# VKoskiv/c-ray

Hardware: AMD Instinct MI355X
Metric: Mray/s (primary+secondary) (higher is better)
Workload: dtype f32; 1 GPU; input/hdr.json 1280x720, 256 spp, 8 bounces (BASELINE.json configs[1]); venusscaled.obj = generated 524288-triangle stand-in (tools/gen_assets.py), HDR env map + 2048^2 grid texture from the reference tree; environment map: a generated stand-in of the HDR's size (tools/cfg2_blob.py — no reference tree to flatten hdr.json from): the same paths and rays, other radiance; parallelism=1 rank: the whole frame in one dispatch

## Files before the change

### c-ray_amd/csrc/cray_hip.hip

```cpp
#include <hip/hip_runtime.h>
#include <dlfcn.h>

#include <algorithm>
#include <chrono>
#include <cmath>
#include <cstdio>
#include <cstring>
#include <condition_variable>
#include <atomic>
#include <cassert>
#include <memory>
#include <mutex>
#include <thread>
#include <string>
#include <vector>

#include "cray_hip.h"
#define CRH_EM_POW_TABLES_IN_LDS
#include "pt_device.h"
#include "scene_compile.h"
#include "ctx_access.h"

using namespace crh;

// ... 6 lines not shown
#endif
#define CRH_INST_LDS_BYTES ((CRH_INST_LDS0_MAX + CRH_INST_LDS1_MAX) * 64u)
#ifndef CRH_SHADE_LDS
#define CRH_SHADE_LDS 1
#endif
#define CRH_SHADE_LDS_MATERIALS 24u
#define CRH_SHADE_LDS_BSDFS 64u
#define CRH_SHADE_LDS_CONSTS 48u
#define CRH_SHADE_LDS_IMAGES 8u
#define CRH_SHADE_LDS_BYTES (CRH_SHADE_LDS * (CRH_SHADE_LDS_MATERIALS * 32u + CRH_SHADE_LDS_BSDFS * 16u + CRH_SHADE_LDS_CONSTS * 16u + CRH_SHADE_LDS_IMAGES * 40u))
#ifndef CRH_STACK_LDS
#define CRH_STACK_LDS ((40960 - 3968 - (int)CRH_INST_LDS_BYTES - (int)CRH_SHADE_LDS_BYTES) / 1024 - 15)
#endif
#ifndef CRH_LOCKSTEP
#define CRH_LOCKSTEP() do { } while (0)
#endif

static thread_local std::string t_err;
static int fail(int code, const std::string &msg) { t_err = msg; return code; }
#define HIP_TRY(expr)                                                                               \
	do {                                                                                            \
		hipError_t e_ = (expr);                                                                     \
		if (e_ != hipSuccess) return fail(CRH_ERR_HIP, std::string(#expr) + ": " + hipGetErrorString(e_)); \
	} while (0)
#include "ctx_buffers.h"

#define CRH_STACK_OVF (134 - CRH_STACK_LDS)
#define CRH_OVF_WORDS_PER_WAVE (128u * 64u)
typedef __attribute__((address_space(3))) uint32_t lds_u32;
typedef __attribute__((address_space(1))) uint32_t glb_u32;
// ... 104 lines not shown
};

template <class T>
__device__ __forceinline__ const T *asGlobal(const T *p) {
	return (const T *)(const __attribute__((address_space(1))) T *)p;
}
__device__ __forceinline__ DScene globalize(const DScene &S) {
	DScene G = S;
	G.nodes = asGlobal(S.nodes); G.tris = asGlobal(S.tris); G.prims = asGlobal(S.prims); G.shade = asGlobal(S.shade);
	G.instances = asGlobal(S.instances); G.materials = asGlobal(S.materials);
	G.bsdfs = asGlobal(S.bsdfs); G.consts = asGlobal(S.consts); G.images = asGlobal(S.images); G.prog = asGlobal(S.prog);
	G.textures = asGlobal(S.textures); G.texels = asGlobal(S.texels);
	G.camera = (const crh_camera *)(const __attribute__((address_space(4))) crh_camera *)S.camera;
	return G;
}

__device__ __forceinline__ uint32_t waveSum(uint32_t v) {
	for (int off = 32; off > 0; off >>= 1) v += __shfl_xor(v, off);
	return v;
}
__device__ __forceinline__ void flushCounter(bool lead, uint32_t laneCount, unsigned long long *counter) {
	const uint32_t v = waveSum(laneCount);
	if (lead && v) atomicAdd(counter, (unsigned long long)v);
}
template <class Cnt>
__device__ __forceinline__ void flushWalkCounters(bool lead, const Cnt &cnt, unsigned long long *counters) {
	flushCounter(lead, cnt.rays, &counters[1]);
	if constexpr (Cnt::level >= 2) {
		flushCounter(lead, cnt.node_tests, &counters[2]);
		flushCounter(lead, cnt.tri_tests, &counters[3]);
// ... 105 lines not shown
		return v;
	}
	__device__ __forceinline__ f4 *at(uint32_t bytes) const { return (f4 *)((char *)base + bytes); }
	__device__ __forceinline__ f4 *rec(uint32_t id) const { return base + id * (LEAN ? 4u : CRH_PATH_F4); }
	__device__ __forceinline__ f4 *hit(uint32_t id) const { return LEAN ? at(vgprConst(CRH_PATHS * 64u) + id * 16u) : base + id * CRH_PATH_F4 + 4u; }
	__device__ __forceinline__ float *inst(uint32_t id) const { return LEAN ? (float *)at(vgprConst(CRH_PATHS * 80u) + id * 4u) : (float *)(base + id * CRH_PATH_F4 + 5u); }
};
static_assert(CRH_PATHS * (4u + 1u) * 4u + CRH_PATHS <= CRH_WAVE_QUEUE_FLOATS, "the lean arrays fit in the wave's table");
static_assert((CRH_WAVE_QUEUE_FLOATS * sizeof(float)) % 64u == 0, "a wave's table starts on a 64-B line when the allocation does, and a lean rec(id) (64 B) is one aligned line: loadRec4 / storeRec4");

__device__ __forceinline__ uint32_t laneRank(unsigned long long m) {
	return __builtin_amdgcn_mbcnt_hi((uint32_t)(m >> 32), __builtin_amdgcn_mbcnt_lo((uint32_t)m, 0u));
}

#if CRH_SHADE_LDS
#define CRH_STAGE_SHADE_TABLES() \
	__shared__ __attribute__((aligned(16))) uint32_t s_shade[CRH_SHADE_LDS_BYTES / 4u]; \
	stk.shadeTab = nullptr; \
	if (S.material_count <= CRH_SHADE_LDS_MATERIALS && S.bsdf_count <= CRH_SHADE_LDS_BSDFS && S.const_count <= CRH_SHADE_LDS_CONSTS && \
		S.image_count <= CRH_SHADE_LDS_IMAGES && S.texture_count <= CRH_SHADE_LDS_IMAGES) { \
		const uint32_t texBase = CRH_SHADE_LDS_MATERIALS * 8u + CRH_SHADE_LDS_BSDFS * 4u + CRH_SHADE_LDS_CONSTS * 4u; \
		for (uint32_t i = threadIdx.x; i < S.texture_count * 8u; i += CRH_BLOCK) s_shade[texBase + i] = ((const uint32_t *)S.textures)[i]; \
		for (uint32_t i = threadIdx.x; i < S.image_count * 2u; i += CRH_BLOCK) s_shade[texBase + CRH_SHADE_LDS_IMAGES * 8u + i] = ((const uint32_t *)S.images)[i]; \
		for (uint32_t i = threadIdx.x; i < S.material_count * 8u; i += CRH_BLOCK) s_shade[i] = ((const uint32_t *)S.materials)[i]; \
		for (uint32_t i = threadIdx.x; i < S.bsdf_count * 4u; i += CRH_BLOCK) s_shade[CRH_SHADE_LDS_MATERIALS * 8u + i] = ((const uint32_t *)S.bsdfs)[i]; \
		for (uint32_t i = threadIdx.x; i < S.const_count * 4u; i += CRH_BLOCK) s_shade[CRH_SHADE_LDS_MATERIALS * 8u + CRH_SHADE_LDS_BSDFS * 4u + i] = ((const uint32_t *)S.consts)[i]; \
		__syncthreads(); \
		stk.shadeTab = (const lds_u32 *)s_shade; \
	}
#else
#define CRH_STAGE_SHADE_TABLES() do { } while (0)
#endif
#if CRH_INST_LDS_BYTES > 0
#define CRH_STAGE_INSTANCE_TABLES() \
	__shared__ __attribute__((aligned(16))) uint32_t s_inst[CRH_INST_LDS_BYTES / 4u]; \
	stk.inst0 = stk.inst1 = nullptr; \
	{ \
		const bool st0 = S.instance_count <= CRH_INST_LDS0_MAX, st1 = S.instance_count <= CRH_INST_LDS1_MAX; \
		if (st0) for (uint32_t i = threadIdx.x; i < S.instance_count * 16u; i += CRH_BLOCK) s_inst[i] = ((const uint32_t *)(S.instances + (i >> 4)))[i & 15u]; \
		if (st1) for (uint32_t i = threadIdx.x; i < S.instance_count * 16u; i += CRH_BLOCK) s_inst[CRH_INST_LDS0_MAX * 16u + i] = ((const uint32_t *)(S.instances + (i >> 4)))[16u + (i & 15u)]; \
		if (st0 || st1) __syncthreads(); \
		if (st0) stk.inst0 = (const lds_u32 *)s_inst; \
		if (st1) stk.inst1 = (const lds_u32 *)s_inst + CRH_INST_LDS0_MAX * 16u; \
	}
#else
#define CRH_STAGE_INSTANCE_TABLES() do { } while (0)
// ... 170 lines not shown
	size_t streamSlots = 0;
	DevBuf<float> dStreamSlab;
	StreamCtl *dStreamCtl = nullptr;
	DevBuf<uint32_t> dStreamOvf;
	unsigned int *hStreamDone = nullptr, *dStreamDone = nullptr;
	unsigned int streamSeq = 0;
	uint64_t streamIterations = 0;
	hipEvent_t streamEv[2] = {nullptr, nullptr};
	uint32_t lastGrid = 0;
	char lastKernel[64] = "";
	DevBuf<float> dStage;
	bool haveScene = false;
	bool hasPrograms = true;
	bool hasVolumes = false;
	DScene d;
	int walk = CRH_WALK_BINARY;
	bool haveWide = false;
	uint32_t wideTlasRoot = 0;
	std::vector<void *> sceneAllocs;
	unsigned long long *dCounters = nullptr;
	uint32_t *dWork = nullptr;
	uint32_t workSlot = 0;
	StagedBuf tileSlots[64];
	std::vector<TimedPair> pendingTimes;
	TimedPool eventPool;
	float lastMs = 0.0f;
	double totalMs = 0.0;
	uint64_t launches = 0;
	uint32_t aovDepth = 0;
	SideDispatch aov;
// ... 14 lines not shown
}

static int watchTimeMs(const char *who, crh_ctx *c, Stopwatch<1> *watch, float *last_ms) {
	if (!c || !last_ms) return fail(CRH_ERR_INVALID, std::string(who) + ": NULL argument");
	int rc = setDevice(c);
	if (rc) return rc;
	if ((rc = watch->read())) return rc;
	*last_ms = watch->sum;
	return CRH_OK;
}

static void freeScene(crh_ctx *c) {
	for (void *p : c->sceneAllocs) (void)hipFree(p);
	c->sceneAllocs.clear();
	c->haveScene = false;
}

static int resolveTimes(crh_ctx *c, bool wait) {
	size_t done = 0;
	for (auto &t : c->pendingTimes) {
		if (wait) HIP_TRY(hipEventSynchronize(t.b));
		else if (hipEventQuery(t.b) != hipSuccess) break;
		float ms = 0.0f;
		HIP_TRY(hipEventElapsedTime(&ms, t.a, t.b));
		c->lastMs = ms;
		c->totalMs += ms;
		c->eventPool.give(t);
		++done;
	}
	c->pendingTimes.erase(c->pendingTimes.begin(), c->pendingTimes.begin() + done);
// ... 81 lines not shown
	CRH_WAVE_ROW(1, 4, true, 0),
#else
	CRH_WAVE_ROW(1, 4, false, 0),
#endif
};
#undef CRH_WAVE_ROW
#endif

static hipError_t launchPathtrace(crh_ctx *c, uint32_t grid, const crh_render_params *P, const BlockQueue &Q, float *dev_fb, int chunk) {
	const int level = c->counterLevel >= 2 ? 2 : 1, samp = c->sampler == CRH_SAMPLER_HALTON ? 1 : 0;
	const char *name = nullptr;
	if (rollForm(c)) {
		const bool wide = wideWalk(c);
		DScene d = c->d;
		if (wide && d.tlas_node_count > 1u) d.tlas_root = c->wideTlasRoot;
		if (const auto *r = pickRow(kRollRows, level, c->hasPrograms, samp, wide ? 1 : 0)) {
			name = r->name;
			hipLaunchKernelGGL((r->fn), dim3(grid), dim3(CRH_BLOCK), 0, c->stream, d, *P, Q, dev_fb, c->dCounters, c->dStage.p, chunk, c->dWaveStats, c->sched, c->dQueues.p, c->dOvf.p, c->dErr);
		}
	}
#ifdef CRH_WITH_ALT_KERNELS
	else if (c->kernel == CRH_KERNEL_WG) {
		if (const auto *r = pickRow(kWgRows, level, c->hasPrograms, samp, 0)) {
			name = r->name;
			hipLaunchKernelGGL((r->fn), dim3(grid), dim3(CRH_BLOCK), 0, c->stream, c->d, *P, Q, dev_fb, c->dCounters, c->dStage.p, chunk, c->schedWg, c->dQueues.p, c->dOvf.p, c->dErr);
		}
	} else if (const auto *r = pickRow(kWaveRows, level, c->hasPrograms, samp, samp || c->wavesPerSimd >= 4 ? 4 : 1)) {
		name = r->name;
		hipLaunchKernelGGL((r->fn), dim3(grid), dim3(CRH_BLOCK), 0, c->stream, c->d, *P, Q, dev_fb, c->dCounters, c->dStage.p, chunk, c->dWaveStats, c->sched, c->dQueues.p, c->dOvf.p);
	}
// ... 71 lines not shown
	crh_ctx *c = new (std::nothrow) crh_ctx();
	if (!c) return fail(CRH_ERR_NOMEM, "out of host memory");
	c->device = device;
	hipError_t e = hipSetDevice(device);
	hipDeviceProp_t prop;
	if (e == hipSuccess) e = hipGetDeviceProperties(&prop, device);
	if (e == hipSuccess) {
		c->cuCount = prop.multiProcessorCount;
		if (stream) c->stream = (hipStream_t)stream;
		else { e = hipStreamCreateWithFlags(&c->stream, hipStreamNonBlocking); c->ownStream = (e == hipSuccess); }
	}
	if (e == hipSuccess) e = hipMalloc((void **)&c->dCounters, CRH_COUNTER_BYTES(c->cuCount));
	if (e == hipSuccess) e = hipMemset(c->dCounters, 0, CRH_COUNTER_BYTES(c->cuCount));
	if (e == hipSuccess) e = hipMalloc((void **)&c->dWork, CRH_WORK_SLOTS * sizeof(uint32_t));
	if (e == hipSuccess) e = hipMemset(c->dWork, 0, CRH_WORK_SLOTS * sizeof(uint32_t));
	if (e == hipSuccess) e = hipHostMalloc((void **)&c->hErr, sizeof(unsigned int), hipHostMallocDefault);
	if (e == hipSuccess) { *c->hErr = 0u; e = hipHostGetDevicePointer((void **)&c->dErr, c->hErr, 0); }
	if (e != hipSuccess) {
		const std::string msg = std::string("crh_context_create: ") + hipGetErrorString(e);
		crh_context_destroy(c);
		return fail(CRH_ERR_HIP, msg);
	}
	const char *env = getenv("CRH_BLOCKS_PER_CU");
	if (env && atoi(env) > 0) c->blocksPerCU = atoi(env) > 8 ? 8 : atoi(env);
	env = getenv("CRH_SWAP_IN_RUN");
	if (env && atoi(env) >= 1 && atoi(env) <= 65) c->sched.swapInRun = atoi(env);
	env = getenv("CRH_KERNEL");
	if (env && !strcmp(env, "stream")) c->kernel = CRH_KERNEL_STREAM;
	if (env && !strcmp(env, "roll")) c->kernel = CRH_KERNEL_ROLL;
	env = getenv("CRH_STREAM_COHORTS");
// ... 13 lines not shown
	}
	if (join && c->janitor.joinable()) c->janitor.join();
}

int crh_context_destroy(crh_ctx *c) {
	if (!c) return CRH_OK;
	(void)hipSetDevice(c->device);
	if (c->stream) (void)hipStreamSynchronize(c->stream);
	freeScene(c);
	auto drop = [](void *p) { if (p) (void)hipFree(p); };
	auto dropEvent = [](hipEvent_t e) { if (e) (void)hipEventDestroy(e); };
	for (StagedBuf &ts : c->tileSlots) ts.release();
	for (const TimedPair &t : c->pendingTimes) c->eventPool.give(t);
	c->pendingTimes.clear();
	c->eventPool.release();
	drop(c->dCounters); drop(c->dWork);
	c->dStage.release(); c->dDefer.release(); c->dQueues.release(); c->dOvf.release();
	for (SideDispatch *s : {&c->aov, &c->ids}) { drop(s->counter); s->tiles.release(); s->watch.release(); }
	c->dPack.release(); c->packWatch.release();
	c->dDenoise.release(); c->denoiseWatch.release();
	c->adaptive.release(); c->adaptiveWatch.release();
	if (c->hErr) (void)hipHostFree(c->hErr);
	if (c->pinned) (void)hipHostFree(c->pinned);
	releaseJanitor(c, true);
	c->dSrgb.release(); c->dGather.release();
	drop(c->dWaveStats); drop(c->dDump);
	for (int i = 0; i < 2; ++i) { drop(c->dProbeHits[i]); drop(c->dProbeInst[i]); }
	drop(c->dProbeOvf); c->dProbeUnits.release();
	c->dStreamPlanes.release(); c->dStreamHit.release(); c->dStreamHitInst.release(); c->dStreamCount.release(); c->dStreamSlab.release();
	drop(c->dStreamCtl); c->dStreamOvf.release();
	if (c->hStreamDone) (void)hipHostFree(c->hStreamDone);
// ... 143 lines not shown
	UP(textures, cs.textures.data(), cs.textures.size());
	{
		void *texDev = nullptr;
		rc = takeTexels ? takeTexels(&texDev) : CRH_OK;
		if (rc) { freeScene(c); return rc; }
		if (texDev) { c->sceneAllocs.push_back(texDev); d.texels = (const f4 *)texDev; }
		else UP(texels, cs.texels.data(), cs.texels.size());
	}
#undef UP
	d.tlas_first = cs.tlas_first;
	d.material_count = (uint32_t)cs.materials.size(); d.bsdf_count = (uint32_t)cs.bsdfs.size(); d.const_count = (uint32_t)cs.consts.size();
	d.image_count = (uint32_t)cs.images.size(); d.texture_count = (uint32_t)cs.textures.size();
	d.tlas_root = cs.tlas_root; d.tlas_node_count = cs.tlas_node_count; d.tlas_prim_base = cs.tlas_prim_base; d.shade_classes = cs.shade_classes; d.instance_count = (uint32_t)cs.instances.size();
	d.background = cs.background;
	{ const crh_camera *cam = nullptr; rc = upload(c, &cs.camera, 1, &cam); if (rc) { freeScene(c); return rc; } d.camera = cam; }
	c->d = d;
	c->haveWide = !cs.wide.empty(); c->wideTlasRoot = cs.wide_tlas_root;
	if (cs.want_wide && !c->haveWide && !cs.wide_refused.empty())
		fprintf(stderr, "libcray_hip: CRH_WALK_WIDE4 was asked for, but this scene has no 4-ary copy (%s): the binary walk renders it\n", cs.wide_refused.c_str());
	c->hasPrograms = cs.prog.size() > 1 || cs.has_volumes || getenv("CRH_FORCE_PROGRAMS") != nullptr;
	c->hasVolumes = cs.has_volumes;
	c->aovDepth = cs.max_albedo_depth;
	c->haveScene = true;
	*tCopiesMs = upMs();
	rc = preloadKernel(c, true);
	if (rc != CRH_OK) return rc;
	unsigned int flag = 0;
	HIP_TRY(hipMemcpy(&flag, c->dWork + (CRH_WORK_SLOTS - 1), sizeof(flag), hipMemcpyDeviceToHost));
	return CRH_OK;
}
// ... 1714 lines not shown
```

### c-ray_amd/csrc/pathtrace_roll.h

```cpp
#pragma once

#define CRH_ROLL_HITS_MAX 136u
#define CRH_ROLL_IDS_MISSES (CRH_IDS_HITS + 2u * CRH_ROLL_HITS_MAX)
#define CRH_ROLL_IDS_BYTES (CRH_ROLL_IDS_MISSES + 128u)
#ifndef CRH_ROLL_SLOTS
#define CRH_ROLL_SLOTS 4u
#endif
#ifndef CRH_ROLL_FIFO
#define CRH_ROLL_FIFO 0
#endif
#define CRH_ROLL_SLOT_SHIFT 30u
#define CRH_ROLL_ITEM_MASK 0x3FFFFFFFu


template <int LEVEL, int WPS, bool PROG, int SAMP, bool WIDE = false>
__global__ __launch_bounds__(CRH_BLOCK, CRH_WPS_OVERRIDE) void k_pathtrace_roll(const DScene Sarg, const crh_render_params P, const BlockQueue Q, float *fb,
																 unsigned long long *counters,
																 float *stage, int chunk, unsigned long long *waveStats, const Sched K, float *queues, uint32_t *ovfAll, unsigned int *errFlag) {
	__shared__ uint32_t s_stack[CRH_STACK_LDS * CRH_BLOCK];
	__shared__ uint32_t s_park[CRH_PARK_SLOTS * CRH_BLOCK];
	enum { RQ_RAYS, RQ_HITS, RQ_MISSES, RQ_FREE, RQ_CLS_LO, RQ_CLS_HI,
	       RQ_GENLEFT,
	       RQ_FLAGS,
	       RQ_HEAD,
// ... 9 lines not shown
#define CRH_RQ_IS_DRY(v) ((v) != 0)
	enum { NS = (int)CRH_ROLL_SLOTS, RQ_WORDS = RQ_SLOT0 + NS * SJ_WORDS };
	static_assert(NS >= 2 && NS <= 4, "2..4 job slots (two bits of the item word)");
	static_assert((CRH_STACK_LDS + CRH_PARK_SLOTS) * CRH_BLOCK * 4 + (CRH_BLOCK / 64) * (CRH_ROLL_IDS_BYTES + RQ_WORDS * 4) + 512 + 256 + CRH_INST_LDS_BYTES + CRH_SHADE_LDS_BYTES <= 40960, "4 blocks per CU share 160 KB of LDS (incl. powf's tables)");
	const DScene S = globalize(Sarg);
	CRH_EM_POW_TABLES_INIT();
	const unsigned long long tStart = wall_clock64();
	uint32_t unitsDone = 0;
#ifdef CRH_EXP_ABS_TIMES
	unsigned long long tDry = 0;
	bool snapDone = false;
#endif
	LdsStack stk;
	stk.lds = (lds_u32 *)&s_stack[threadIdx.x];
	stk.parkp = (lds_u32 *)&s_park[threadIdx.x];
	CRH_STAGE_SHADE_TABLES();
	CRH_STAGE_INSTANCE_TABLES();
	CountersT<LEVEL, PROG, WIDE> cnt;
	memset(&cnt, 0, sizeof(cnt));
	const uint32_t lane = threadIdx.x & 63u;
	const uint32_t wave = (blockIdx.x * CRH_BLOCK + threadIdx.x) >> 6;
	__shared__ uint8_t s_cls[256];
	const bool sorted = K.sortFrom > 0 && S.shade_classes >= (uint32_t)K.sortFrom && S.instance_count <= 256u;
	if (sorted) {
		for (uint32_t i = threadIdx.x; i < S.instance_count; i += CRH_BLOCK) s_cls[i] = (uint8_t)CRH_DINST_CLASS(S.instances[i].kind);
		__syncthreads();
	}
	stk.ovf = (glb_u32 *)ovfAll + (size_t)__builtin_amdgcn_readfirstlane(wave) * CRH_OVF_WORDS_PER_WAVE;
	const size_t slabFloats = (size_t)Q.bw * Q.bh * chunk * 3;
	float *const myStage = stage + (size_t)__builtin_amdgcn_readfirstlane(wave) * (size_t)NS * slabFloats;
	const int passEnd = P.first_pass + P.pass_count;
	const uint32_t trisOff = (uint32_t)((const char *)S.tris - (const char *)S.nodes);
	constexpr bool LEANTAB = CRH_PATH_LEAN && !PROG;
	constexpr bool COOP_LOAD = LEANTAB && CRH_REC_COOP_LOAD == 1, COOP_LOAD_MISS = LEANTAB && CRH_REC_COOP_LOAD >= 1 , COOP_STORE = LEANTAB && CRH_REC_COOP_STORE, MISS_SKIP_HIT = LEANTAB && CRH_MISS_SKIP_HIT;
	const PathTab<LEANTAB> tab{(f4 *)(queues + (size_t)__builtin_amdgcn_readfirstlane(wave) * CRH_WAVE_QUEUE_FLOATS)};
	unsigned long long *const waveCtr = counters + CRH_NCOUNTERS + (size_t)__builtin_amdgcn_readfirstlane(wave) * CRH_NCOUNTERS;
	float *dumpRays = nullptr;
	uint32_t dumpCap = 0, dumpCount = 0;
	if constexpr (LEVEL >= 2) {
		if (waveStats) {
			const unsigned long long base = waveStats[CRH_DUMP_HDR];
			if (base) { dumpCap = (uint32_t)waveStats[CRH_DUMP_HDR + 1]; dumpRays = (float *)(__attribute__((address_space(1))) float *)(uintptr_t)base + (size_t)__builtin_amdgcn_readfirstlane(wave) * dumpCap * 6u; }
		}
	}
#define CRH_WCTR(k, v) atomicAdd(&waveCtr[k], (unsigned long long)(uint32_t)(v))
	__shared__ int s_rq[(CRH_BLOCK / 64) * RQ_WORDS];
	__shared__ __attribute__((aligned(2))) uint8_t s_ids[(CRH_BLOCK / 64) * CRH_ROLL_IDS_BYTES];
	typedef volatile __attribute__((address_space(3))) int lds_int;
// ... 25 lines not shown
			if (left < 0) left = 0;
			moreChunks = !(gj[SJ_WH] & SJ_WH_DEFER) && gj[SJ_PASS0] + gj[SJ_PASSN] < passEnd;
			if (oj[SJ_NEXT] >= (ob & 0xFFFF) * (ob >> 16) * oj[SJ_PASSN] && oj[SJ_OUT] == 0 && (open > 1 || !moreChunks)) flags |= 1;
		}
		if (open < NS && (!CRH_RQ_IS_DRY(wq[RQ_DRY]) || moreChunks)) flags |= 2;
		wq[RQ_GENLEFT] = left; wq[RQ_FLAGS] = flags;
	};

	if (lane == 0) {
		wq[RQ_RAYS] = 0; wq[RQ_HITS] = 0; wq[RQ_MISSES] = 0; wq[RQ_FREE] = (int)CRH_PATHS; wq[RQ_CLS_LO] = 0; wq[RQ_CLS_HI] = 0;
		wq[RQ_HEAD] = 0; wq[RQ_OPEN] = 0; wq[RQ_GEN] = 0; wq[RQ_DRY] = 0;
		for (int i = 0; i < NS * SJ_WORDS; ++i) wq[RQ_SLOT0 + i] = 0;
		refreshJobWords();
	}
	for (uint32_t i = lane; i < CRH_PATHS; i += 64u) ids[i] = (uint8_t)i;
	__threadfence_block();
	Walk w;
	memset(&w, 0, sizeof(w));
	w.phase = PH_IDLE;
	uint32_t myPath = 0;
	auto retireRefill = [&](int &rq, int &hq, int &mq) __attribute__((always_inline)) {
		const bool fin = (w.phase == PH_SHADE);
		const bool finHit = fin && w.hit.inst >= 0, finMiss = fin && w.hit.inst < 0;
		const unsigned long long hm = __ballot(finHit), mm = __ballot(finMiss);
		uint32_t cls = 0;
		if (fin) {
			if (!MISS_SKIP_HIT || finHit) *tab.hit(myPath) = f4{w.hit.t, w.hit.u, w.hit.v, asF32((uint32_t)w.hit.slot)};
			if (finHit) {
				*tab.inst(myPath) = asF32((uint32_t)w.hit.inst);
				if (sorted) cls = (uint32_t)((volatile __attribute__((address_space(3))) uint8_t *)s_cls)[w.hit.inst];
				hits[(uint32_t)hq + laneRank(hm)] = (uint16_t)(myPath | (cls << 8));
// ... 30 lines not shown
			myPath = myRay;
#else
		if (idle && (int)er < take) {
			myPath = ids[CRH_IDS_RAYS + (uint32_t)(rq - take) + er];
#endif
			const f4 *q = tab.rec(myPath);
			const f4 q0 = q[0], q1 = q[1];
			{ TablePort<SAMP> port2{tab.rec(myPath)}; walkBegin(S, w, stk, v3{q0.x, q0.y, q0.z}, v3{q1.x, q1.y, q1.z}, cnt, port2, (uint32_t)K.rayFlags); }
			if constexpr (LEVEL >= 2) {
				if (dumpRays && dumpCount + er < dumpCap) { float *o = dumpRays + (size_t)(dumpCount + er) * 6u; o[0] = q0.x; o[1] = q0.y; o[2] = q0.z; o[3] = q1.x; o[4] = q1.y; o[5] = q1.z; }
			}
		}
		if constexpr (LEVEL >= 2) dumpCount += (uint32_t)take;
		hq += (int)__popcll(hm); mq += (int)__popcll(mm); rq -= take;
		if (lane == 0) { wq[RQ_HITS] = hq; wq[RQ_MISSES] = mq; wq[RQ_RAYS] = rq; }
		__threadfence_block();
	};
	uint32_t guard = (uint32_t)K.roundLimit;
	for (;;) {
		if (--guard == 0u) { if (lane == 0) atomicOr(errFlag, CRH_ERRFLAG_ROUND_LIMIT); break; }
#ifdef CRH_EXP_ABS_TIMES
		if (waveStats && !snapDone && (guard & 15u) == 0u) {
			uint32_t handedOut = 0;
			if (lane == 0) handedOut = __hip_atomic_load((uint32_t *)Q.counter, __ATOMIC_RELAXED, __HIP_MEMORY_SCOPE_AGENT);
			handedOut = __builtin_amdgcn_readfirstlane(handedOut);
			if (handedOut >= Q.total) {
				snapDone = true;
				if (lane == 0) {
					const int head = wq[RQ_HEAD], open = wq[RQ_OPEN];
					unsigned long long notGenerated = 0, notStaged = 0;
					for (int k = 0; k < open; ++k) {
// ... 59 lines not shown
					if constexpr (LEVEL >= 2) {
						if (lane == 0) { CRH_WCTR(11, 1); CRH_WCTR(17, now); }
#ifdef CRH_CENSUS
						const uint32_t wf = (uint32_t)__popcll(__ballot(w.phase == PH_SHADE || w.phase == PH_IDLE));
						if (lane == 0) { CRH_WCTR(30, nTw >= K.triInRun ? 0u : (uint32_t)nTw); CRH_WCTR(31, wf); if (nTw >= K.triInRun) { CRH_WCTR(26, 1); CRH_WCTR(27, nTw); } }
#endif
					}
					if (isN || isT) {
						const uint32_t off = isN ? (uint32_t)(w.node << (WIDE ? 4 : 5)) : trisOff + w.pA * 48u;
						const char *rec = (const char *)S.nodes + off;
						q0 = *(const f4 *)rec; q1 = *(const f4 *)(rec + 16); q2 = *(const f4 *)(rec + 32); q3 = *(const f4 *)(rec + 48);
						if (WIDE || isT) { q4 = *(const f4 *)(rec + 64); q5 = *(const f4 *)(rec + 80); }
						if (WIDE && isN) { q6 = *(const f4 *)(rec + 96); q7 = *(const f4 *)(rec + 112); }
					}
					if constexpr (WIDE) { if (isN) stepWideLoaded<true>(S, w, stk, cnt, port, q0, q1, q2, q3, q4, q5, q6, q7); }
					else
					if (isN) stepNodeLoaded<true>(S, w, stk, cnt, port, q0, q1, q2, q3);
					if (isT) stepTriLoaded(S, w, stk, cnt, port, q0, q1, q2, q3, q4, q5);
					if ((int)__popcll(__ballot(w.phase == PH_CTRL)) >= K.ctrlInRun) {
#ifdef CRH_CENSUS
						if constexpr (LEVEL >= 2) { const uint32_t n2 = (uint32_t)__popcll(__ballot(w.phase == PH_CTRL)); if (lane == 0) { CRH_WCTR(28, 1); CRH_WCTR(29, n2); } }
#endif
						if (w.phase == PH_CTRL) stepCtrl(S, w, stk, cnt, port);
					}
					{
						const int nFi = (int)__popcll(__ballot(w.phase == PH_SHADE)), nEi = (int)__popcll(__ballot(w.phase == PH_IDLE));
						if (nFi + nEi >= K.swapInRun && (nFi > 0 || rqRun > 0) && hqRun < 64 && mqRun < 64) {
							if constexpr (LEVEL >= 2) { if (lane == 0) { CRH_WCTR(21, 1); CRH_WCTR(23, nFi + min(nEi + nFi, rqRun)); } }
							retireRefill(rqRun, hqRun, mqRun);
							port = TablePort<SAMP>{tab.rec(myPath)};
						}
					}
					now = __popcll(__ballot(w.phase == PH_NODE));
// ... 67 lines not shown
					if (have) {
						lds_int *j = wq + RQ_SLOT0 + s * SJ_WORDS;
						j[SJ_X0] = J.x0; j[SJ_Y0] = J.y0; j[SJ_WH] = J.w | (J.h << 16) | defer
						          ; j[SJ_BWBH] = J.bw | (J.bh << 16); j[SJ_PASS0] = J.passBegin; j[SJ_PASSN] = J.passCount;
						j[SJ_NEXT] = 0; j[SJ_OUT] = 0;
						j[SJ_BASE_LO] = (int)(uint32_t)(uintptr_t)base; j[SJ_BASE_HI] = (int)(uint32_t)((uintptr_t)base >> 32);
						wq[RQ_OPEN] = open + 1; wq[RQ_GEN] = s;
					} else {
						wq[RQ_DRY] = 1;
					}
#ifdef CRH_EXP_ABS_TIMES
					if (!have && !tDry) tDry = wall_clock64();
#endif
					refreshJobWords();
				}
				__threadfence_block();
				break;
			}
			case ST_GEN: {
				const int g = wq[RQ_GEN];
				const BlockJob J = loadJob(g);
				const uint32_t genNext = (uint32_t)wq[RQ_SLOT0 + g * SJ_WORDS + SJ_NEXT], genItems = genNext + (uint32_t)itemsLeft;
				const uint32_t item = genNext + lane;
				int x = 0, y = 0, pass = 0;
				const bool valid = item < genItems && decodeItem(J, item, x, y, pass);
				const unsigned long long vm = __ballot(valid);
				const int n = (int)__popcll(vm);
				if constexpr (COOP_STORE) {
					f4 q0 = f4{0.0f, 0.0f, 0.0f, 0.0f}, q1 = q0, q2 = q0, q3 = q0;
					uint32_t id = 0;
					if (valid) {
// ... 10 lines not shown
				if (valid) {
					const uint32_t rk = laneRank(vm);
					const uint32_t id = ids[CRH_IDS_FREE_END - (uint32_t)freeQ + rk];
					v3 ro, rd;
					PathRecT<RngT<SAMP>> r;
					beginPath(S, P, x, y, pass, ro, rd, r, cnt);
					putPathRay(tab.rec(id), ro, rd, r, item | ((uint32_t)g << CRH_ROLL_SLOT_SHIFT));
					ids[CRH_IDS_RAYS + (uint32_t)raysQ + rk] = (uint8_t)id;
				}
				if (lane == 0) {
					wq[RQ_RAYS] = raysQ + n; wq[RQ_FREE] = freeQ - n;
					lds_int *j = wq + RQ_SLOT0 + g * SJ_WORDS;
					j[SJ_NEXT] = (int)(genNext + 64u); j[SJ_OUT] = j[SJ_OUT] + n;
					refreshJobWords();
				}
				__threadfence_block();
				break;
			}
			case ST_MISS: {
				const int n = min(missQn, 64);
				int mySlot = -1;
				const bool have = (int)lane < n;
				uint32_t id = 0;
				f4 q0, q1, q2, q3;
				if constexpr (COOP_LOAD_MISS) {
					if (have) id = ids[CRH_ROLL_IDS_MISSES + (uint32_t)(missQn - n) + lane];
					tab.loadRec4(id, have, q0, q1, q2, q3);
				}
				if (have) {
					if constexpr (!COOP_LOAD_MISS) { id = ids[CRH_ROLL_IDS_MISSES + (uint32_t)(missQn - n) + lane]; const f4 *q = tab.rec(id); q1 = q[1]; q2 = q[2]; q3 = q[3]; }
					v3 ro{0.0f, 0.0f, 0.0f}, rd{q1.x, q1.y, q1.z};
					PathRecT<RngT<SAMP>> r;
					r.wr = q2.x; r.wg = q2.y; r.wb = q2.z;
					r.fr = q3.x; r.fg = q3.y; r.fb = q3.z;
					r.rng.state = 0; r.depth = 0;
					const uint32_t item = asU32(q1.w);
					mySlot = (int)(item >> CRH_ROLL_SLOT_SHIFT);
					TravHit h;
					h.t = MISS_SKIP_HIT ? 0.0f : tab.hit(id)->x; h.u = h.v = 0.0f; h.slot = -1; h.inst = -1;
					(void)shadeCore(S, P, ro, rd, h, r, cnt, stk);
					float *so = sampleSlot(mySlot, item & CRH_ROLL_ITEM_MASK); so[0] = r.fr; so[1] = r.fg; so[2] = r.fb;
					ids[CRH_IDS_FREE_END - 1u - (uint32_t)freeQ - lane] = (uint8_t)id;
				}
				int fin[NS];
#pragma unroll
				for (int s = 0; s < NS; ++s) fin[s] = (int)__popcll(__ballot(mySlot == s));
				if (lane == 0) {
					wq[RQ_MISSES] = missQn - n; wq[RQ_FREE] = freeQ + n;
#pragma unroll
					for (int s = 0; s < NS; ++s) if (fin[s]) wq[RQ_SLOT0 + s * SJ_WORDS + SJ_OUT] = wq[RQ_SLOT0 + s * SJ_WORDS + SJ_OUT] - fin[s];
					refreshJobWords();
				}
				__threadfence_block();
				break;
			}
			case ST_FOLD: {
				const int o = wq[RQ_HEAD], open = wq[RQ_OPEN];
				const BlockJob J = loadJob(o);
				__threadfence_block();
				const float *slab = myStage + (size_t)o * slabFloats;
				if (!jobDeferred(o)) {
					for (uint32_t pix = lane; pix < (uint32_t)(J.bw * J.bh); pix += 64u) foldBlockPixel(P, J, pix, slab, fb);
				}
				__threadfence_block();
				CRH_LOCKSTEP();
				if (lane == 0) { wq[RQ_HEAD] = (o + 1) % NS; wq[RQ_OPEN] = open - 1; refreshJobWords(); }
				__threadfence_block();
				break;
			}
			default: {
				uint32_t clsLo = 0, clsHi = 0;
				int n = min(hitsQ, 64);
				if (sorted) {
				clsLo = (uint32_t)__builtin_amdgcn_readfirstlane(wq[RQ_CLS_LO]); clsHi = (uint32_t)__builtin_amdgcn_readfirstlane(wq[RQ_CLS_HI]);
				int c8[8];
#pragma unroll
				for (int b = 0; b < 8; ++b) c8[b] = (int)(((b < 4 ? clsLo : clsHi) >> (8 * (b & 3))) & 255u);
				uint32_t fullMask = 0;
				int partCls = -1, partN = 0;
				n = 0;
#pragma unroll
				for (int it = 0; it < 8; ++it) {
// ... 54 lines not shown
					if constexpr (!COOP_LOAD) id = (uint32_t)hits[(uint32_t)(hitsQ - n) + lane] & 255u;
					f4 *q = tab.rec(id);
					if constexpr (!COOP_LOAD) { q0 = q[0]; q1 = q[1]; q2 = q[2]; q3 = q[3]; }
					const f4 q4 = *tab.hit(id);
					v3 ro{q0.x, q0.y, q0.z}, rd{q1.x, q1.y, q1.z};
					PathRecT<RngT<SAMP>> r;
					r.wr = q2.x; r.wg = q2.y; r.wb = q2.z;
					r.fr = q3.x; r.fg = q3.y; r.fb = q3.z;
					r.rng.state = (uint64_t)asU32(q2.w) | ((uint64_t)asU32(q3.w) << 32);
					r.depth = (int)asU32(q0.w);
					const uint32_t item = asU32(q1.w);
					TravHit h;
					h.t = q4.x; h.u = q4.y; h.v = q4.z;
					h.slot = (int32_t)asU32(q4.w); h.inst = (int32_t)asU32(*tab.inst(id));
					__builtin_assume(h.inst >= 0);
					cont = shadeCore(S, P, ro, rd, h, r, cnt, stk);
					done = !cont;
					if constexpr (COOP_STORE) packPathRay(q0, q1, q2, q3, ro, rd, r, item);
					else if (cont) putPathRay(q, ro, rd, r, item);
					if (!cont) {
						mySlot = (int)(item >> CRH_ROLL_SLOT_SHIFT);
						float *so = sampleSlot(mySlot, item & CRH_ROLL_ITEM_MASK); so[0] = r.fr; so[1] = r.fg; so[2] = r.fb;
					}
				}
				if constexpr (COOP_STORE) tab.storeRec4(id, cont, q0, q1, q2, q3);
				const unsigned long long cm = __ballot(cont), dm = __ballot(done);
				int fin[NS];
#pragma unroll
				for (int s = 0; s < NS; ++s) fin[s] = (int)__popcll(__ballot(mySlot == s));
				if (cont) ids[CRH_IDS_RAYS + (uint32_t)raysQ + laneRank(cm)] = (uint8_t)id;
				if (done) ids[CRH_IDS_FREE_END - 1u - (uint32_t)freeQ - laneRank(dm)] = (uint8_t)id;
				if (lane == 0) {
					const int nd = (int)__popcll(dm);
					wq[RQ_HITS] = hitsQ - n; wq[RQ_RAYS] = raysQ + (int)__popcll(cm); wq[RQ_FREE] = freeQ + nd;
					wq[RQ_CLS_LO] = (int)clsLo; wq[RQ_CLS_HI] = (int)clsHi;
#pragma unroll
					for (int s = 0; s < NS; ++s) if (fin[s]) wq[RQ_SLOT0 + s * SJ_WORDS + SJ_OUT] = wq[RQ_SLOT0 + s * SJ_WORDS + SJ_OUT] - fin[s];
					if (nd) refreshJobWords();
				}
				__threadfence_block();
				break;
			}
		}
		if constexpr (LEVEL >= 2) {
			if (lane == 0) {
				const uint32_t dt = CRH_TICK() - tk;
				CRH_WCTR(14, 1);
				if (pick == ST_NODE) { CRH_WCTR(9, dt); }
				else if (pick == ST_TRI) { CRH_WCTR(8, dt); }
				else if (pick == ST_CTRL) { CRH_WCTR(13, 1); CRH_WCTR(16, dt); CRH_WCTR(25, nC); }
				else if (pick == ST_SWAP) { CRH_WCTR(21, 1); CRH_WCTR(19, dt); CRH_WCTR(23, nF + min(nE + nF, raysQ)); }
				else if (pick == ST_GEN || pick == ST_MISS || pick == ST_OPEN || pick == ST_FOLD) { CRH_WCTR(22, 1); CRH_WCTR(20, dt); }
				else { CRH_WCTR(15, 1); CRH_WCTR(10, dt); }
			}
		}
// ... 22 lines not shown
```

### c-ray_amd/csrc/pt_device.h

```cpp
#pragma once
#include <stdint.h>
#include <math.h>
#include <float.h>
#include <type_traits>
#include <utility>
#include "cray_hip.h"
#include "exact_math.h"

#if defined(__HIPCC__)
#define CRH_DEV __device__ __forceinline__
#define CRH_DEV_NOINLINE __device__ __noinline__
#define CRH_MEM __device__ __forceinline__
#else
#define CRH_MEM inline __attribute__((always_inline))
#define CRH_DEV static inline __attribute__((always_inline))
#define CRH_DEV_NOINLINE static __attribute__((noinline))
#endif

namespace crh {

#define CRH_PI 3.141592653589793238462643383279502f
#define CRH_NONE 0xFFFFFFFFu

struct alignas(16) f4 { float x, y, z, w; };
// ... 74 lines not shown
	const f4 *consts;
	const DImage *images;
	const DOp *prog;
	const DTexture *textures;
	const f4 *texels;
	uint32_t tlas_root;
	uint32_t tlas_node_count;
	uint32_t tlas_prim_base;
	uint32_t background;
	uint32_t shade_classes;
	uint32_t instance_count;
	uint32_t image_count, texture_count;
	uint32_t material_count, bsdf_count, const_count;
	uint32_t tlas_first;
	const crh_camera *camera;
};

template <int LEVEL, bool PROGRAMS, bool WIDE = false> struct CountersT;
template <bool PROGRAMS, bool WIDE> struct CountersT<2, PROGRAMS, WIDE> {
	static constexpr int level = 2;
	static constexpr bool programs = PROGRAMS;
	static constexpr bool wide = WIDE;
	uint32_t rays, node_tests, tri_tests, inst_visits, inst_hits, sphere_tests, tex_fetches, paths;
	uint32_t t_setup, t_trav, t_shade;
	uint32_t w_node, w_tri, w_ctrl, w_round, w_shade, w_setup;
	uint32_t u_node, u_shade;
	uint32_t t_swap, t_gen, n_swap, n_gen, u_swap, u_tri, u_ctrl;
#ifdef CRH_CENSUS
	uint32_t w_tri_in, u_tri_in, w_ctrl_in, u_ctrl_in;
	uint32_t u_wait_tri, u_wait_fin;
// ... 792 lines not shown
	CRH_COUNT1(cnt, rays, 1);
	w.k = makeRayK(o, d);
	w.k.oct |= rayFlags;
	if (S.tlas_node_count < 1u) { w.phase = PH_SHADE; return; }
	if (S.tlas_node_count == 1u) {
		const f4 n0 = S.nodes[2u * S.tlas_root], n1 = S.nodes[2u * S.tlas_root + 1u];
		float tE;
		CRH_COUNT(cnt, node_tests, 1);
		if (intersectNode(n0, n1, w.k, w.hit.t, tE)) { w.pA = CRH_DNODE_FIRST(n1); w.pAe = w.pA + CRH_DNODE_COUNT(n1); }
	} else {
		w.node = S.tlas_root;
	}
	walkAdvance(S, w, stk, cnt, port);
}

template <bool FAST = true, class Stack, class Cnt, class Port>
CRH_DEV void stepNodeLoaded(const DScene &S, Walk &w, Stack &stk, Cnt &cnt, Port &port, const f4 l0, const f4 l1, const f4 r0, const f4 r1) {
	float tL, tR;
	CRH_COUNT(cnt, node_tests, 2);
	const bool hitL = intersectNode<FAST>(l0, l1, w.k, w.hit.t, tL);
	const bool hitR = intersectNode<FAST>(r0, r1, w.k, w.hit.t, tR);
	const bool leafL = CRH_DNODE_ISLEAF(l1), leafR = CRH_DNODE_ISLEAF(r1);
	const uint32_t fl = CRH_DNODE_FIRST(l1), fr = CRH_DNODE_FIRST(r1);
	const bool lL = hitL && leafL, lR = hitR && leafR;
	const uint32_t nL = lL ? CRH_DNODE_COUNT(l1) : 0u, nR = lR ? CRH_DNODE_COUNT(r1) : 0u;
	w.pA = lL ? fl : fr;
	w.pAe = w.pA + (lL ? nL : nR);
	w.pB = fr;
	w.pBe = fr + (lL ? nR : 0u);
	const bool inL = hitL && !leafL, inR = hitR && !leafR;
	const bool swap = tL > tR;
	if (inL && inR) stk.push(w.sp++, swap ? fl : fr);
	w.node = (inL && inR) ? (swap ? fr : fl) : (inL ? fl : (inR ? fr : CRH_NONE));
	walkAdvance(S, w, stk, cnt, port);
}
template <bool FAST = true, class Stack, class Cnt, class Port>
CRH_DEV void stepNode(const DScene &S, Walk &w, Stack &stk, Cnt &cnt, Port &port) {
	const char *pair = (const char *)S.nodes + (uint32_t)(w.node << 5);
	const f4 l0 = *(const f4 *)pair, l1 = *(const f4 *)(pair + 16), r0 = *(const f4 *)(pair + 32), r1 = *(const f4 *)(pair + 48);
	stepNodeLoaded<FAST>(S, w, stk, cnt, port, l0, l1, r0, r1);
}

template <bool FAST = true, class Stack, class Cnt, class Port>
CRH_DEV void stepWideLoaded(const DScene &S, Walk &w, Stack &stk, Cnt &cnt, Port &port, const f4 a0, const f4 a1, const f4 b0, const f4 b1, const f4 c0, const f4 c1, const f4 d0, const f4 d1) {
	float t0, t1, t2, t3;
	CRH_COUNT(cnt, node_tests, 4);
	const bool h0 = intersectNode<FAST>(a0, a1, w.k, w.hit.t, t0);
	const bool h1 = intersectNode<FAST>(b0, b1, w.k, w.hit.t, t1);
// ... 29 lines not shown

template <class Cnt>
CRH_DEV void testTriangle(const f4 q0, const f4 q1, const f4 q2, uint32_t slot, Walk &w, Cnt &cnt) {
	const v3 v0 = v3{q0.x, q0.y, q0.z}, e1 = v3{q0.w, q1.x, q1.y}, e2 = v3{q1.z, q1.w, q2.x}, n = v3{q2.y, q2.z, q2.w};
	CRH_COUNT(cnt, tri_tests, 1);
	const v3 c = vsub(v0, w.k.o);
	const v3 r = vcross(w.k.d, c);
	const float invDet = 1.0f / vdot(n, w.k.d);
	const float u = vdot(r, e2) * invDet;
	const float v = vdot(r, e1) * invDet;
	if (u >= 0.0f && v >= 0.0f && u + v <= 1.0f) {
		const float t = vdot(n, c) * invDet;
		if (t >= 0.0f && t < w.hit.t) { w.hit.t = t; w.hit.u = u; w.hit.v = v; w.hit.slot = (int32_t)slot; w.instFound = 1; }
	}
}
template <class Stack, class Cnt, class Port>
CRH_DEV void stepTriLoaded(const DScene &S, Walk &w, Stack &stk, Cnt &cnt, Port &port, const f4 a0, const f4 a1, const f4 a2, const f4 b0, const f4 b1, const f4 b2) {
	const uint32_t slot = w.pA;
	const bool two = slot + 1u < w.pAe;
	const uint32_t slot2 = two ? slot + 1u : slot;
	w.pA = slot2 + 1u;
	if (w.pA == w.pAe) { w.pA = w.pB; w.pAe = w.pBe; w.pB = w.pBe = 0; }
	testTriangle(a0, a1, a2, slot, w, cnt);
	if (two) testTriangle(b0, b1, b2, slot2, w, cnt);
	walkAdvance(S, w, stk, cnt, port);
}
template <class Stack, class Cnt, class Port>
CRH_DEV void stepTri(const DScene &S, Walk &w, Stack &stk, Cnt &cnt, Port &port) {
	const uint32_t slot = w.pA;
	const uint32_t slot2 = slot + 1u < w.pAe ? slot + 1u : slot;
	const char *ta = (const char *)S.tris + (uint32_t)(slot * 48u), *tb = (const char *)S.tris + (uint32_t)(slot2 * 48u);
	const f4 a0 = *(const f4 *)ta, a1 = *(const f4 *)(ta + 16), a2 = *(const f4 *)(ta + 32);
	const f4 b0 = *(const f4 *)tb, b1 = *(const f4 *)(tb + 16), b2 = *(const f4 *)(tb + 32);
	stepTriLoaded(S, w, stk, cnt, port, a0, a1, a2, b0, b1, b2);
}

template <class Stack, class Cnt, class Port>
CRH_DEV void stepCtrl(const DScene &S, Walk &w, Stack &stk, Cnt &cnt, Port &port) {
	const uint32_t slot = w.pA++;
// ... 301 lines not shown
```

Baseline: 9160 Mray/s.

## Merge traversal advance, move shade args to constant buffer, use wave-scope fences

Splits the node and triangle step functions into test-only parts so the binary walk calls walkAdvance once after either test instead of inlining it twice. Shading scene pointers move into a separate device-side DShadeArgs struct, loaded through the constant address space at shade time, so fewer scene fields stay live across traversal. Block-scope thread fences are replaced with wavefront-scope fences, which are cheaper because all the queue state is per-wave. Each part is behind its own macro, and the change risks extra scalar loads at each shade call and relies on wave-scope ordering being enough.

```diff
diff --git a/c-ray_amd/csrc/cray_hip.hip b/c-ray_amd/csrc/cray_hip.hip
--- a/c-ray_amd/csrc/cray_hip.hip
+++ b/c-ray_amd/csrc/cray_hip.hip
@@ -44,6 +44,20 @@
 #endif
 #ifndef CRH_LOCKSTEP
 #define CRH_LOCKSTEP() do { } while (0)
+#endif
+#ifndef CRH_MERGED_ADVANCE
+#define CRH_MERGED_ADVANCE 1
+#endif
+#ifndef CRH_STEP_ARGS
+#define CRH_STEP_ARGS 1
+#endif
+#ifndef CRH_WAVE_SCOPE_FENCE
+#define CRH_WAVE_SCOPE_FENCE 1
+#endif
+#if CRH_WAVE_SCOPE_FENCE
+#define CRH_WAVE_FENCE() __builtin_amdgcn_fence(__ATOMIC_SEQ_CST, "wavefront")
+#else
+#define CRH_WAVE_FENCE() __threadfence_block()
 #endif
 
 static thread_local std::string t_err;
@@ -178,6 +192,19 @@
 	G.camera = (const crh_camera *)(const __attribute__((address_space(4))) crh_camera *)S.camera;
 	return G;
 }
+__device__ __forceinline__ DScene shadeScene(const DScene &S) {
+#if CRH_STEP_ARGS
+	const __attribute__((address_space(4))) DShadeArgs *a = (const __attribute__((address_space(4))) DShadeArgs *)S.shadeArgs;
+	DScene G = S;
+	G.shade = asGlobal(a->shade); G.materials = asGlobal(a->materials); G.bsdfs = asGlobal(a->bsdfs); G.consts = asGlobal(a->consts); G.images = asGlobal(a->images);
+	G.prog = asGlobal(a->prog); G.textures = asGlobal(a->textures); G.texels = asGlobal(a->texels);
+	G.background = a->background; G.image_count = a->image_count; G.texture_count = a->texture_count;
+	G.material_count = a->material_count; G.bsdf_count = a->bsdf_count; G.const_count = a->const_count;
+	return G;
+#else
+	return S;
+#endif
+}
 
 __device__ __forceinline__ uint32_t waveSum(uint32_t v) {
 	for (int off = 32; off > 0; off >>= 1) v += __shfl_xor(v, off);
@@ -313,22 +340,24 @@
 }
 
 #if CRH_SHADE_LDS
-#define CRH_STAGE_SHADE_TABLES() \
+#define CRH_STAGE_SHADE_TABLES() CRH_STAGE_SHADE_TABLES_OF(S)
+#define CRH_STAGE_SHADE_TABLES_OF(SCENE) \
 	__shared__ __attribute__((aligned(16))) uint32_t s_shade[CRH_SHADE_LDS_BYTES / 4u]; \
 	stk.shadeTab = nullptr; \
-	if (S.material_count <= CRH_SHADE_LDS_MATERIALS && S.bsdf_count <= CRH_SHADE_LDS_BSDFS && S.const_count <= CRH_SHADE_LDS_CONSTS && \
-		S.image_count <= CRH_SHADE_LDS_IMAGES && S.texture_count <= CRH_SHADE_LDS_IMAGES) { \
+	if ((SCENE).material_count <= CRH_SHADE_LDS_MATERIALS && (SCENE).bsdf_count <= CRH_SHADE_LDS_BSDFS && (SCENE).const_count <= CRH_SHADE_LDS_CONSTS && \
+		(SCENE).image_count <= CRH_SHADE_LDS_IMAGES && (SCENE).texture_count <= CRH_SHADE_LDS_IMAGES) { \
 		const uint32_t texBase = CRH_SHADE_LDS_MATERIALS * 8u + CRH_SHADE_LDS_BSDFS * 4u + CRH_SHADE_LDS_CONSTS * 4u; \
-		for (uint32_t i = threadIdx.x; i < S.texture_count * 8u; i += CRH_BLOCK) s_shade[texBase + i] = ((const uint32_t *)S.textures)[i]; \
-		for (uint32_t i = threadIdx.x; i < S.image_count * 2u; i += CRH_BLOCK) s_shade[texBase + CRH_SHADE_LDS_IMAGES * 8u + i] = ((const uint32_t *)S.images)[i]; \
-		for (uint32_t i = threadIdx.x; i < S.material_count * 8u; i += CRH_BLOCK) s_shade[i] = ((const uint32_t *)S.materials)[i]; \
-		for (uint32_t i = threadIdx.x; i < S.bsdf_count * 4u; i += CRH_BLOCK) s_shade[CRH_SHADE_LDS_MATERIALS * 8u + i] = ((const uint32_t *)S.bsdfs)[i]; \
-		for (uint32_t i = threadIdx.x; i < S.const_count * 4u; i += CRH_BLOCK) s_shade[CRH_SHADE_LDS_MATERIALS * 8u + CRH_SHADE_LDS_BSDFS * 4u + i] = ((const uint32_t *)S.consts)[i]; \
+		for (uint32_t i = threadIdx.x; i < (SCENE).texture_count * 8u; i += CRH_BLOCK) s_shade[texBase + i] = ((const uint32_t *)(SCENE).textures)[i]; \
+		for (uint32_t i = threadIdx.x; i < (SCENE).image_count * 2u; i += CRH_BLOCK) s_shade[texBase + CRH_SHADE_LDS_IMAGES * 8u + i] = ((const uint32_t *)(SCENE).images)[i]; \
+		for (uint32_t i = threadIdx.x; i < (SCENE).material_count * 8u; i += CRH_BLOCK) s_shade[i] = ((const uint32_t *)(SCENE).materials)[i]; \
+		for (uint32_t i = threadIdx.x; i < (SCENE).bsdf_count * 4u; i += CRH_BLOCK) s_shade[CRH_SHADE_LDS_MATERIALS * 8u + i] = ((const uint32_t *)(SCENE).bsdfs)[i]; \
+		for (uint32_t i = threadIdx.x; i < (SCENE).const_count * 4u; i += CRH_BLOCK) s_shade[CRH_SHADE_LDS_MATERIALS * 8u + CRH_SHADE_LDS_BSDFS * 4u + i] = ((const uint32_t *)(SCENE).consts)[i]; \
 		__syncthreads(); \
 		stk.shadeTab = (const lds_u32 *)s_shade; \
 	}
 #else
 #define CRH_STAGE_SHADE_TABLES() do { } while (0)
+#define CRH_STAGE_SHADE_TABLES_OF(SCENE) do { } while (0)
 #endif
 #if CRH_INST_LDS_BYTES > 0
 #define CRH_STAGE_INSTANCE_TABLES() \
@@ -529,6 +558,7 @@
 	bool hasPrograms = true;
 	bool hasVolumes = false;
 	DScene d;
+	DShadeArgs *dNoShadeArgs = nullptr;
 	int walk = CRH_WALK_BINARY;
 	bool haveWide = false;
 	uint32_t wideTlasRoot = 0;
@@ -573,6 +603,7 @@
 	for (void *p : c->sceneAllocs) (void)hipFree(p);
 	c->sceneAllocs.clear();
 	c->haveScene = false;
+	c->d = DScene{};
 }
 
 static int resolveTimes(crh_ctx *c, bool wait) {
@@ -684,6 +715,7 @@
 		const bool wide = wideWalk(c);
 		DScene d = c->d;
 		if (wide && d.tlas_node_count > 1u) d.tlas_root = c->wideTlasRoot;
+		if (!d.shadeArgs) d.shadeArgs = c->dNoShadeArgs;
 		if (const auto *r = pickRow(kRollRows, level, c->hasPrograms, samp, wide ? 1 : 0)) {
 			name = r->name;
 			hipLaunchKernelGGL((r->fn), dim3(grid), dim3(CRH_BLOCK), 0, c->stream, d, *P, Q, dev_fb, c->dCounters, c->dStage.p, chunk, c->dWaveStats, c->sched, c->dQueues.p, c->dOvf.p, c->dErr);
@@ -785,6 +817,8 @@
 	if (e == hipSuccess) e = hipMemset(c->dCounters, 0, CRH_COUNTER_BYTES(c->cuCount));
 	if (e == hipSuccess) e = hipMalloc((void **)&c->dWork, CRH_WORK_SLOTS * sizeof(uint32_t));
 	if (e == hipSuccess) e = hipMemset(c->dWork, 0, CRH_WORK_SLOTS * sizeof(uint32_t));
+	if (e == hipSuccess) e = hipMalloc((void **)&c->dNoShadeArgs, sizeof(DShadeArgs));
+	if (e == hipSuccess) e = hipMemset(c->dNoShadeArgs, 0, sizeof(DShadeArgs));
 	if (e == hipSuccess) e = hipHostMalloc((void **)&c->hErr, sizeof(unsigned int), hipHostMallocDefault);
 	if (e == hipSuccess) { *c->hErr = 0u; e = hipHostGetDevicePointer((void **)&c->dErr, c->hErr, 0); }
 	if (e != hipSuccess) {
@@ -828,7 +862,7 @@
 	for (const TimedPair &t : c->pendingTimes) c->eventPool.give(t);
 	c->pendingTimes.clear();
 	c->eventPool.release();
-	drop(c->dCounters); drop(c->dWork);
+	drop(c->dCounters); drop(c->dWork); drop(c->dNoShadeArgs);
 	c->dStage.release(); c->dDefer.release(); c->dQueues.release(); c->dOvf.release();
 	for (SideDispatch *s : {&c->aov, &c->ids}) { drop(s->counter); s->tiles.release(); s->watch.release(); }
 	c->dPack.release(); c->packWatch.release();
@@ -1002,6 +1036,12 @@
 	d.tlas_root = cs.tlas_root; d.tlas_node_count = cs.tlas_node_count; d.tlas_prim_base = cs.tlas_prim_base; d.shade_classes = cs.shade_classes; d.instance_count = (uint32_t)cs.instances.size();
 	d.background = cs.background;
 	{ const crh_camera *cam = nullptr; rc = upload(c, &cs.camera, 1, &cam); if (rc) { freeScene(c); return rc; } d.camera = cam; }
+	{
+		const DShadeArgs sa{d.shade, d.materials, d.bsdfs, d.consts, d.images, d.prog, d.textures, d.texels, d.background, d.image_count, d.texture_count, d.material_count, d.bsdf_count, d.const_count};
+		const DShadeArgs *dev = nullptr;
+		rc = upload(c, &sa, 1, &dev); if (rc) { freeScene(c); return rc; }
+		d.shadeArgs = dev;
+	}
 	c->d = d;
 	c->haveWide = !cs.wide.empty(); c->wideTlasRoot = cs.wide_tlas_root;
 	if (cs.want_wide && !c->haveWide && !cs.wide_refused.empty())
diff --git a/c-ray_amd/csrc/pathtrace_roll.h b/c-ray_amd/csrc/pathtrace_roll.h
--- a/c-ray_amd/csrc/pathtrace_roll.h
+++ b/c-ray_amd/csrc/pathtrace_roll.h
@@ -47,7 +47,8 @@
 	LdsStack stk;
 	stk.lds = (lds_u32 *)&s_stack[threadIdx.x];
 	stk.parkp = (lds_u32 *)&s_park[threadIdx.x];
-	CRH_STAGE_SHADE_TABLES();
+	const DScene Sstage = shadeScene(S);
+	CRH_STAGE_SHADE_TABLES_OF(Sstage);
 	CRH_STAGE_INSTANCE_TABLES();
 	CountersT<LEVEL, PROG, WIDE> cnt;
 	memset(&cnt, 0, sizeof(cnt));
@@ -65,6 +66,7 @@
 	const int passEnd = P.first_pass + P.pass_count;
 	const uint32_t trisOff = (uint32_t)((const char *)S.tris - (const char *)S.nodes);
 	constexpr bool LEANTAB = CRH_PATH_LEAN && !PROG;
+	constexpr bool MERGED_ADVANCE = CRH_MERGED_ADVANCE != 0;
 	constexpr bool COOP_LOAD = LEANTAB && CRH_REC_COOP_LOAD == 1, COOP_LOAD_MISS = LEANTAB && CRH_REC_COOP_LOAD >= 1 , COOP_STORE = LEANTAB && CRH_REC_COOP_STORE, MISS_SKIP_HIT = LEANTAB && CRH_MISS_SKIP_HIT;
 	const PathTab<LEANTAB> tab{(f4 *)(queues + (size_t)__builtin_amdgcn_readfirstlane(wave) * CRH_WAVE_QUEUE_FLOATS)};
 	unsigned long long *const waveCtr = counters + CRH_NCOUNTERS + (size_t)__builtin_amdgcn_readfirstlane(wave) * CRH_NCOUNTERS;
@@ -120,7 +122,7 @@
 		refreshJobWords();
 	}
 	for (uint32_t i = lane; i < CRH_PATHS; i += 64u) ids[i] = (uint8_t)i;
-	__threadfence_block();
+	CRH_WAVE_FENCE();
 	Walk w;
 	memset(&w, 0, sizeof(w));
 	w.phase = PH_IDLE;
@@ -181,7 +183,7 @@
 		if constexpr (LEVEL >= 2) dumpCount += (uint32_t)take;
 		hq += (int)__popcll(hm); mq += (int)__popcll(mm); rq -= take;
 		if (lane == 0) { wq[RQ_HITS] = hq; wq[RQ_MISSES] = mq; wq[RQ_RAYS] = rq; }
-		__threadfence_block();
+		CRH_WAVE_FENCE();
 	};
 	uint32_t guard = (uint32_t)K.roundLimit;
 	for (;;) {
@@ -271,9 +273,13 @@
 						if (WIDE && isN) { q6 = *(const f4 *)(rec + 96); q7 = *(const f4 *)(rec + 112); }
 					}
 					if constexpr (WIDE) { if (isN) stepWideLoaded<true>(S, w, stk, cnt, port, q0, q1, q2, q3, q4, q5, q6, q7); }
-					else
+					else if constexpr (MERGED_ADVANCE) {
+						if (isN) stepNodeTest<true>(w, stk, cnt, q0, q1, q2, q3);
+						if (isT) stepTriTest(w, cnt, q0, q1, q2, q3, q4, q5);
+						if (isN || isT) walkAdvance(S, w, stk, cnt, port);
+					} else
 					if (isN) stepNodeLoaded<true>(S, w, stk, cnt, port, q0, q1, q2, q3);
-					if (isT) stepTriLoaded(S, w, stk, cnt, port, q0, q1, q2, q3, q4, q5);
+					if constexpr (WIDE || !MERGED_ADVANCE) { if (isT) stepTriLoaded(S, w, stk, cnt, port, q0, q1, q2, q3, q4, q5); }
 					if ((int)__popcll(__ballot(w.phase == PH_CTRL)) >= K.ctrlInRun) {
 #ifdef CRH_CENSUS
 						if constexpr (LEVEL >= 2) { const uint32_t n2 = (uint32_t)__popcll(__ballot(w.phase == PH_CTRL)); if (lane == 0) { CRH_WCTR(28, 1); CRH_WCTR(29, n2); } }
@@ -371,7 +377,7 @@
 #endif
 					refreshJobWords();
 				}
-				__threadfence_block();
+				CRH_WAVE_FENCE();
 				break;
 			}
 			case ST_GEN: {
@@ -412,7 +418,7 @@
 					j[SJ_NEXT] = (int)(genNext + 64u); j[SJ_OUT] = j[SJ_OUT] + n;
 					refreshJobWords();
 				}
-				__threadfence_block();
+				CRH_WAVE_FENCE();
 				break;
 			}
 			case ST_MISS: {
@@ -436,7 +442,7 @@
 					mySlot = (int)(item >> CRH_ROLL_SLOT_SHIFT);
 					TravHit h;
 					h.t = MISS_SKIP_HIT ? 0.0f : tab.hit(id)->x; h.u = h.v = 0.0f; h.slot = -1; h.inst = -1;
-					(void)shadeCore(S, P, ro, rd, h, r, cnt, stk);
+					(void)shadeCore(shadeScene(S), P, ro, rd, h, r, cnt, stk);
 					float *so = sampleSlot(mySlot, item & CRH_ROLL_ITEM_MASK); so[0] = r.fr; so[1] = r.fg; so[2] = r.fb;
 					ids[CRH_IDS_FREE_END - 1u - (uint32_t)freeQ - lane] = (uint8_t)id;
 				}
@@ -449,21 +455,21 @@
 					for (int s = 0; s < NS; ++s) if (fin[s]) wq[RQ_SLOT0 + s * SJ_WORDS + SJ_OUT] = wq[RQ_SLOT0 + s * SJ_WORDS + SJ_OUT] - fin[s];
 					refreshJobWords();
 				}
-				__threadfence_block();
+				CRH_WAVE_FENCE();
 				break;
 			}
 			case ST_FOLD: {
 				const int o = wq[RQ_HEAD], open = wq[RQ_OPEN];
 				const BlockJob J = loadJob(o);
-				__threadfence_block();
+				CRH_WAVE_FENCE();
 				const float *slab = myStage + (size_t)o * slabFloats;
 				if (!jobDeferred(o)) {
 					for (uint32_t pix = lane; pix < (uint32_t)(J.bw * J.bh); pix += 64u) foldBlockPixel(P, J, pix, slab, fb);
 				}
-				__threadfence_block();
+				CRH_WAVE_FENCE();
 				CRH_LOCKSTEP();
 				if (lane == 0) { wq[RQ_HEAD] = (o + 1) % NS; wq[RQ_OPEN] = open - 1; refreshJobWords(); }
-				__threadfence_block();
+				CRH_WAVE_FENCE();
 				break;
 			}
 			default: {
@@ -548,7 +554,7 @@
 					h.t = q4.x; h.u = q4.y; h.v = q4.z;
 					h.slot = (int32_t)asU32(q4.w); h.inst = (int32_t)asU32(*tab.inst(id));
 					__builtin_assume(h.inst >= 0);
-					cont = shadeCore(S, P, ro, rd, h, r, cnt, stk);
+					cont = shadeCore(shadeScene(S), P, ro, rd, h, r, cnt, stk);
 					done = !cont;
 					if constexpr (COOP_STORE) packPathRay(q0, q1, q2, q3, ro, rd, r, item);
 					else if (cont) putPathRay(q, ro, rd, r, item);
@@ -572,7 +578,7 @@
 					for (int s = 0; s < NS; ++s) if (fin[s]) wq[RQ_SLOT0 + s * SJ_WORDS + SJ_OUT] = wq[RQ_SLOT0 + s * SJ_WORDS + SJ_OUT] - fin[s];
 					if (nd) refreshJobWords();
 				}
-				__threadfence_block();
+				CRH_WAVE_FENCE();
 				break;
 			}
 		}
diff --git a/c-ray_amd/csrc/pt_device.h b/c-ray_amd/csrc/pt_device.h
--- a/c-ray_amd/csrc/pt_device.h
+++ b/c-ray_amd/csrc/pt_device.h
@@ -112,6 +112,18 @@
 	uint32_t material_count, bsdf_count, const_count;
 	uint32_t tlas_first;
 	const crh_camera *camera;
+	const struct DShadeArgs *shadeArgs;
+};
+struct DShadeArgs {
+	const DShadeTri *shade;
+	const crh_material *materials;
+	const DBsdf *bsdfs;
+	const f4 *consts;
+	const DImage *images;
+	const DOp *prog;
+	const DTexture *textures;
+	const f4 *texels;
+	uint32_t background, image_count, texture_count, material_count, bsdf_count, const_count;
 };
 
 template <int LEVEL, bool PROGRAMS, bool WIDE = false> struct CountersT;
@@ -934,8 +946,8 @@
 	walkAdvance(S, w, stk, cnt, port);
 }
 
-template <bool FAST = true, class Stack, class Cnt, class Port>
-CRH_DEV void stepNodeLoaded(const DScene &S, Walk &w, Stack &stk, Cnt &cnt, Port &port, const f4 l0, const f4 l1, const f4 r0, const f4 r1) {
+template <bool FAST = true, class Stack, class Cnt>
+CRH_DEV void stepNodeTest(Walk &w, Stack &stk, Cnt &cnt, const f4 l0, const f4 l1, const f4 r0, const f4 r1) {
 	float tL, tR;
 	CRH_COUNT(cnt, node_tests, 2);
 	const bool hitL = intersectNode<FAST>(l0, l1, w.k, w.hit.t, tL);
@@ -952,6 +964,10 @@
 	const bool swap = tL > tR;
 	if (inL && inR) stk.push(w.sp++, swap ? fl : fr);
 	w.node = (inL && inR) ? (swap ? fr : fl) : (inL ? fl : (inR ? fr : CRH_NONE));
+}
+template <bool FAST = true, class Stack, class Cnt, class Port>
+CRH_DEV void stepNodeLoaded(const DScene &S, Walk &w, Stack &stk, Cnt &cnt, Port &port, const f4 l0, const f4 l1, const f4 r0, const f4 r1) {
+	stepNodeTest<FAST>(w, stk, cnt, l0, l1, r0, r1);
 	walkAdvance(S, w, stk, cnt, port);
 }
 template <bool FAST = true, class Stack, class Cnt, class Port>
@@ -1011,8 +1027,8 @@
 		if (t >= 0.0f && t < w.hit.t) { w.hit.t = t; w.hit.u = u; w.hit.v = v; w.hit.slot = (int32_t)slot; w.instFound = 1; }
 	}
 }
-template <class Stack, class Cnt, class Port>
-CRH_DEV void stepTriLoaded(const DScene &S, Walk &w, Stack &stk, Cnt &cnt, Port &port, const f4 a0, const f4 a1, const f4 a2, const f4 b0, const f4 b1, const f4 b2) {
+template <class Cnt>
+CRH_DEV void stepTriTest(Walk &w, Cnt &cnt, const f4 a0, const f4 a1, const f4 a2, const f4 b0, const f4 b1, const f4 b2) {
 	const uint32_t slot = w.pA;
 	const bool two = slot + 1u < w.pAe;
 	const uint32_t slot2 = two ? slot + 1u : slot;
@@ -1020,6 +1036,10 @@
 	if (w.pA == w.pAe) { w.pA = w.pB; w.pAe = w.pBe; w.pB = w.pBe = 0; }
 	testTriangle(a0, a1, a2, slot, w, cnt);
 	if (two) testTriangle(b0, b1, b2, slot2, w, cnt);
+}
+template <class Stack, class Cnt, class Port>
+CRH_DEV void stepTriLoaded(const DScene &S, Walk &w, Stack &stk, Cnt &cnt, Port &port, const f4 a0, const f4 a1, const f4 a2, const f4 b0, const f4 b1, const f4 b2) {
+	stepTriTest(w, cnt, a0, a1, a2, b0, b1, b2);
 	walkAdvance(S, w, stk, cnt, port);
 }
 template <class Stack, class Cnt, class Port>
```

Result: faster. 9301 Mray/s, median of 6 (+1.5%).
